# jiahuei/COMIC-Compact-Image-Captioning-with-Attention

Hardware: AMD Instinct MI355X
Metric: images/sec (decoder-mode XE training, COMIC-256, InceptionV3 frozen) (higher is better)
Workload: dtype bf16

## Files before the change

### comic-compact-image-captioning-with-attention_amd/csrc/gemm_group.hip

```cpp
#include <algorithm>

#include "gemm_group.h"
#include "gemm_x3_dev.h"

namespace {

constexpr int GB = 128;
constexpr int kGemmGroupSlots = 512;
constexpr int kItemOverhead = 6;
constexpr int kSc1 = 16;
typedef __attribute__((ext_vector_type(4))) unsigned gg_u32x4_t;

__device__ __forceinline__ __amdgpu_buffer_rsrc_t gg_rsrc(const void* p, long bytes) {
  return __builtin_amdgcn_make_buffer_rsrc((void*)p, 0, (int)bytes, 0x00020000);
}
__device__ __forceinline__ float4 gg_load16_sc1(__amdgpu_buffer_rsrc_t r, unsigned off) {
  const gg_u32x4_t v = __builtin_amdgcn_raw_buffer_load_b128(r, (int)off, 0, kSc1);
  return make_float4(__uint_as_float(v.x), __uint_as_float(v.y), __uint_as_float(v.z), __uint_as_float(v.w));
}
__device__ __forceinline__ void gg_store16_sc1(__amdgpu_buffer_rsrc_t r, unsigned off, float4 v) {
  const gg_u32x4_t u = {__float_as_uint(v.x), __float_as_uint(v.y), __float_as_uint(v.z), __float_as_uint(v.w)};
  __builtin_amdgcn_raw_buffer_store_b128(u, r, (int)off, 0, kSc1);
}

constexpr int kGroupLds = 4 * (X3Tile<GB, true>::BYTES + X3Tile<GB, true>::BYTES);
static_assert(X3Tile<GB, true>::BYTES >= X3Tile<GB, false>::BYTES, "LDS of the k-contiguous form bounds the others");
constexpr int kGroupLdsPc = 2 * 2 * (X3TilePc<GB, false>::BYTES + X3TilePc<GB, false>::BYTES);
static_assert(X3TilePc<GB, false>::BYTES >= X3TilePc<GB, true>::BYTES, "LDS of the row-contiguous form bounds the others");

__device__ __forceinline__ void gg_emit(const ComicGemmProb& p, int m, int n, float4 a) {
  if (m >= p.M || n >= p.N) return;
  const int nv = min(4, p.N - n);
  float v[4] = {a.x * p.alpha, a.y * p.alpha, a.z * p.alpha, a.w * p.alpha};
  float* cp = p.C + (size_t)m * p.ldc + n;
#pragma unroll
  for (int q = 0; q < 4; ++q) {
    if (q >= nv) break;
    if (p.bias) v[q] += p.bias[n + q];
    if (p.mask) v[q] = (v[q] / p.keep) * p.mask[(size_t)m * p.ld_mask + n + q];
    if (p.beta != 0.f) v[q] += p.beta * cp[q];
  }
  if (nv == 4 && (p.ldc % 4 == 0) && (((uintptr_t)p.C & 15) == 0)) {
    *(float4*)cp = make_float4(v[0], v[1], v[2], v[3]);
  } else {
#pragma unroll
    for (int q = 0; q < 4; ++q)
      if (q < nv) cp[q] = v[q];
  }
}

template <int FORM>
__global__ __launch_bounds__(FORM == 1 ? 256 : 512)
#if defined(__HIP_DEVICE_COMPILE__)
__attribute__((amdgpu_waves_per_eu(FORM == 3 ? 4 : 1, FORM == 3 ? 4 : 2)))
#endif
void gemm_group_x3_kernel(ComicGemmGroup g) {
  constexpr bool PC = FORM != 1;
  constexpr int NT = PC ? 512 : 256;
  constexpr int LDS = PC ? kGroupLdsPc : kGroupLds;
  extern __shared__ __attribute__((aligned(16))) unsigned char smem[];
  int bid = blockIdx.x;
  if (g.xcd_chunk > 0 && bid < g.xcd_chunk * 8) bid = (bid & 7) * g.xcd_chunk + (bid >> 3);
  volatile unsigned* s_last = (volatile unsigned*)(smem + LDS - 16);
  int pi = 0;
#pragma unroll 1
  for (int i = 1; i < g.n; ++i)
    if (bid >= g.p[i].wg_begin) pi = i;
  const ComicGemmProb& p = g.p[pi];
  const int local = bid - p.wg_begin;
  const int S = p.S, ntiles = p.tiles_m * p.tiles_n;
  const int slice = local / ntiles, tl = local - slice * ntiles;
  constexpr int PW = 8;
  const int panel = tl / (p.tiles_m * PW), rem = tl - panel * p.tiles_m * PW;
  const int pw = min(PW, p.tiles_n - panel * PW);
  const int mt = rem / pw, nt = panel * PW + rem % pw;
  const int tile = mt * p.tiles_n + nt;
  const int m0 = mt * GB, n0 = nt * GB;
  const int kbeg = S > 1 ? slice * p.k_per_slice : 0;
  const int kend = S > 1 ? min(p.K, kbeg + p.k_per_slice) : p.K;
  const int tid = threadIdx.x, lane = tid & 63, wave = tid >> 6;
  const int wm = wave >> 1, wn = wave & 1;

  const long tile_id = (long)p.ticket0 + tile;
  const __amdgpu_buffer_rsrc_t sr = gg_rsrc(g.slab + ((long)p.slab_tile0 + (long)tile * S) * (GB * GB), (long)S * GB * GB * 4);
  const unsigned sbase = (unsigned)slice * (GB * GB * 4);
  if (p.ones_a) {
    constexpr int KG = 8;
    float4* red = (float4*)smem;
    const int cg = tid & 31, kg = tid >> 5, n = n0 + 4 * cg;
    const bool vec = (p.ldb % 4 == 0) && (((uintptr_t)p.B & 15) == 0);
    float4 sm = make_float4(0.f, 0.f, 0.f, 0.f);
    if (n < p.N && kg < KG)
      for (int k = kbeg + kg; k < kend; k += KG) {
        const float4 v = load4(p.B + (size_t)k * p.ldb + n, p.N - n, vec);
        sm.x += v.x; sm.y += v.y; sm.z += v.z; sm.w += v.w;
      }
    if (kg < KG) red[kg * 32 + cg] = sm;
    __syncthreads();
    if (tid < 32) {
      float4 tot = red[cg];
#pragma unroll
      for (int k = 1; k < KG; ++k) {
        const float4 v = red[k * 32 + cg];
        tot.x += v.x; tot.y += v.y; tot.z += v.z; tot.w += v.w;
      }
      if (S == 1) gg_emit(p, 0, n, tot);
      else gg_store16_sc1(sr, sbase + (unsigned)cg * 16u, tot);
    }
    if (S == 1) return;
  } else {
    f32x4_t acc[4][4];
    if constexpr (PC) {
      constexpr int DEPTH = FORM == 3 ? 2 : 4;
      if (p.type == COMIC_GG_TN) x3_mainloop_pc<false, false, DEPTH>(p.A, p.B, p.M, p.N, p.lda, p.ldb, m0, n0, kbeg, kend, smem, acc);
      else if (p.type == COMIC_GG_NN) x3_mainloop_pc<true, false, DEPTH>(p.A, p.B, p.M, p.N, p.lda, p.ldb, m0, n0, kbeg, kend, smem, acc);
      else x3_mainloop_pc<true, true, DEPTH>(p.A, p.B, p.M, p.N, p.lda, p.ldb, m0, n0, kbeg, kend, smem, acc);
    } else {
      if (p.type == COMIC_GG_TN)
        x3_mainloop<GB, false, false, GB>(p.A, p.B, p.M, p.N, p.lda, p.ldb, m0, n0, kbeg, kend, smem, acc);
      else if (p.type == COMIC_GG_NN)
        x3_mainloop<GB, true, false, GB>(p.A, p.B, p.M, p.N, p.lda, p.ldb, m0, n0, kbeg, kend, smem, acc);
      else
        x3_mainloop<GB, true, true, GB>(p.A, p.B, p.M, p.N, p.lda, p.ldb, m0, n0, kbeg, kend, smem, acc);
    }
    const bool owner = wave < 4;
    if (S == 1) {
      if (owner)
#pragma unroll
      for (int i = 0; i < 4; ++i)
#pragma unroll
        for (int j = 0; j < 4; ++j)
          gg_emit(p, m0 + wm * 64 + j * 16 + (lane & 15), n0 + wn * 64 + i * 16 + (lane >> 4) * 4,
                  make_float4(acc[i][j][0], acc[i][j][1], acc[i][j][2], acc[i][j][3]));
      return;
    }
    if (owner)
#pragma unroll
    for (int i = 0; i < 4; ++i)
#pragma unroll
      for (int j = 0; j < 4; ++j) {
        const int ml = wm * 64 + j * 16 + (lane & 15), nl = wn * 64 + i * 16 + (lane >> 4) * 4;
        gg_store16_sc1(sr, sbase + (unsigned)(ml * GB + nl) * 4u, make_float4(acc[i][j][0], acc[i][j][1], acc[i][j][2], acc[i][j][3]));
      }
  }
  asm volatile("s_waitcnt vmcnt(0)" ::: "memory");
  __syncthreads();
  if (tid == 0) {
    const unsigned t = __hip_atomic_fetch_add(g.tickets + tile_id, 1u, __ATOMIC_RELAXED, __HIP_MEMORY_SCOPE_AGENT);
    *s_last = (t == (unsigned)(S - 1)) ? 1u : 0u;
    if (t == (unsigned)(S - 1)) __hip_atomic_store(g.tickets + tile_id, 0u, __ATOMIC_RELAXED, __HIP_MEMORY_SCOPE_AGENT);
  }
  __syncthreads();
  if (!*s_last) return;
  const int n_chunks = p.ones_a ? 1 : (GB * GB / 4) / NT;
#pragma unroll 1
  for (int c = 0; c < n_chunks; c += 4) {
    float4 sum[4];
#pragma unroll
    for (int u = 0; u < 4; ++u) sum[u] = make_float4(0.f, 0.f, 0.f, 0.f);
#pragma unroll 1
    for (int s = 0; s < S; ++s) {
      float4 v[4];
#pragma unroll
      for (int u = 0; u < 4; ++u) v[u] = gg_load16_sc1(sr, (unsigned)s * (GB * GB * 4) + (unsigned)(tid + NT * (c + u)) * 16u);
#pragma unroll
      for (int u = 0; u < 4; ++u) {
        sum[u].x += v[u].x; sum[u].y += v[u].y; sum[u].z += v[u].z; sum[u].w += v[u].w;
      }
    }
#pragma unroll
    for (int u = 0; u < 4; ++u) {
      const int idx4 = tid + NT * (c + u);
      if (!p.ones_a || idx4 < GB / 4) gg_emit(p, m0 + idx4 / (GB / 4), n0 + (idx4 % (GB / 4)) * 4, sum[u]);
    }
  }
}


}

int comic_gemm_group_plan(ComicGemmGroup& g, int target_items, int64_t* slab_bytes, int* n_tickets) {
  COMIC_REQUIRE(g.n > 0 && g.n <= kGemmGroupMax, "gemm_group: %d problems", g.n);
  long cost = 0;
  for (int i = 0; i < g.n; ++i) {
    ComicGemmProb& p = g.p[i];
    COMIC_REQUIRE(p.M > 0 && p.N > 0 && p.K > 0 && p.B && p.C && (p.A || p.ones_a), "gemm_group: bad problem %d", i);
    COMIC_REQUIRE(p.type >= COMIC_GG_TN && p.type <= COMIC_GG_NT, "gemm_group: bad type of problem %d", i);
    COMIC_REQUIRE(!p.ones_a || (p.type == COMIC_GG_TN && p.M == 1), "gemm_group: ones_a needs type TN and M = 1 (problem %d)", i);
    COMIC_REQUIRE(p.ldc >= p.N && (!p.mask || p.ld_mask >= p.N), "gemm_group: leading dimension of problem %d", i);
    if (!p.ones_a) COMIC_REQUIRE(p.lda >= (p.type == COMIC_GG_TN ? p.M : p.K), "gemm_group: lda of problem %d", i);
    COMIC_REQUIRE(p.ldb >= (p.type == COMIC_GG_NT ? p.K : p.N), "gemm_group: ldb of problem %d", i);
    p.tiles_m = cdiv(p.M, GB);
    p.tiles_n = cdiv(p.N, GB);
    cost += (long)cdiv(p.M, GB) * p.tiles_n * cdiv(p.K, 32);
  }
  auto split_of = [](int kt, long klen) { return (int)std::min<long>(16, std::max<long>(1, (kt + klen / 2) / klen)); };
  long klen = std::max<long>(8, cost / std::max(1, target_items));
  {
    long best = -1, best_klen = klen, kt_max = 8;
    for (int i = 0; i < g.n; ++i) kt_max = std::max<long>(kt_max, cdiv(g.p[i].K, 32));
    for (long kl = klen; kl <= kt_max; ++kl) {
      long items = 0, longest = 0;
      for (int i = 0; i < g.n; ++i) {
        const ComicGemmProb& p = g.p[i];
        const int kt = cdiv(p.K, 32), S = split_of(kt, kl);
        items += (long)p.tiles_m * p.tiles_n * S;
        if (!p.ones_a) longest = std::max<long>(longest, cdiv(kt, S));
      }
      const long est = cdiv64(items, kGemmGroupSlots) * (longest + kItemOverhead);
      if (best < 0 || est < best) {
        best = est;
        best_klen = kl;
      }
    }
    klen = best_klen;
  }
  int wg = 0, tickets = 0, slab_tiles = 0;
  for (int i = 0; i < g.n; ++i) {
    ComicGemmProb& p = g.p[i];
    const int nt = cdiv(p.M, GB) * p.tiles_n, kt = cdiv(p.K, 32);
    int S = split_of(kt, klen);
    p.k_per_slice = cdiv(kt, S) * 32;
    S = cdiv(p.K, p.k_per_slice);
    p.S = S;
    p.wg_begin = wg;
    p.slab_tile0 = slab_tiles;
    p.ticket0 = tickets;
    wg += nt * S;
    if (S > 1) {
      slab_tiles += nt * S;
      tickets += nt;
    }
  }
  if (slab_bytes) *slab_bytes = (int64_t)slab_tiles * GB * GB * 4;
  if (n_tickets) *n_tickets = tickets;
  return wg;
}

namespace {
bool gg_vec_ok(const ComicGemmGroup& g) {
  for (int i = 0; i < g.n; ++i) {
    const ComicGemmProb& p = g.p[i];
    if (p.ones_a) continue;
    const bool a_kc = p.type != COMIC_GG_TN, b_kc = p.type == COMIC_GG_NT;
    if (!(p.lda % 4 == 0 && p.ldb % 4 == 0 && ((uintptr_t)p.A & 15) == 0 && ((uintptr_t)p.B & 15) == 0 &&
          (!(a_kc || b_kc) || p.K % 4 == 0)))
      return false;
  }
  return true;
}
const void* gg_kernel(int form) {
  return form == 1 ? (const void*)gemm_group_x3_kernel<1> : form == 2 ? (const void*)gemm_group_x3_kernel<2> : (const void*)gemm_group_x3_kernel<3>;
}
int gg_lds(int form) { return form == 1 ? kGroupLds : kGroupLdsPc; }
int gg_reserve_lds(int form) {
  static PerDeviceOnce once[3];
  bool& done = once[form - 1].slot();
  if (!done) {
    COMIC_REQUIRE(hipFuncSetAttribute(gg_kernel(form), hipFuncAttributeMaxDynamicSharedMemorySize, gg_lds(form)) == hipSuccess,
                  "gemm_group: cannot reserve %d bytes of LDS", gg_lds(form));
    done = true;
  }
  return 0;
}
}

int comic_gemm_group_launch(const ComicGemmGroup& g_in, int n_wg, hipStream_t st, int form) {
  ComicGemmGroup g = g_in;
  g.xcd_chunk = n_wg / 8;
  COMIC_REQUIRE(n_wg > 0, "gemm_group: empty launch");
  COMIC_REQUIRE(form >= 0 && form <= 3, "gemm_group: form %d", form);
  const bool vec = gg_vec_ok(g);
  if (form == 0) form = vec ? 3 : 1;
  COMIC_REQUIRE(form == 1 || vec, "gemm_group: form %d needs 16-byte loadable operands", form);
  if (int rc = gg_reserve_lds(form)) return rc;
  if (form == 1) hipLaunchKernelGGL(gemm_group_x3_kernel<1>, dim3((unsigned)n_wg), dim3(256), kGroupLds, st, g);
  else if (form == 2) hipLaunchKernelGGL(gemm_group_x3_kernel<2>, dim3((unsigned)n_wg), dim3(512), kGroupLdsPc, st, g);
  else hipLaunchKernelGGL(gemm_group_x3_kernel<3>, dim3((unsigned)n_wg), dim3(512), kGroupLdsPc, st, g);
  COMIC_LAUNCH_CHECK("gemm_group");
  return 0;
}

namespace {
int gg_from_public(const comic_gemm_prob* probs, int n, ComicGemmGroup& g) {
  COMIC_REQUIRE(probs && n > 0 && n <= kGemmGroupMax, "gemm_group: 1..%d problems", kGemmGroupMax);
  g = ComicGemmGroup{};
  g.n = n;
  for (int i = 0; i < n; ++i) {
    const comic_gemm_prob& q = probs[i];
    ComicGemmProb& p = g.p[i];
    p.A = q.A; p.B = q.B; p.C = q.C; p.bias = q.bias; p.mask = q.mask;
    p.M = q.M; p.N = q.N; p.K = q.K; p.lda = q.lda; p.ldb = q.ldb; p.ldc = q.ldc; p.ld_mask = q.ld_mask;
    p.alpha = q.alpha; p.beta = q.beta; p.keep = q.keep; p.type = q.type; p.ones_a = q.ones_a;
  }
  return 0;
}
#define kPublicTarget kGemmGroupTargetItems
}

extern "C" int64_t comic_gemm_group_workspace(const comic_gemm_prob* probs, int n) {
  ComicGemmGroup g;
  if (gg_from_public(probs, n, g)) return -1;
  int64_t slab = 0;
  int nt = 0;
  if (comic_gemm_group_plan(g, kPublicTarget, &slab, &nt) < 0) return -1;
  return slab + 256 + (int64_t)nt * 4;
}

extern "C" int comic_gemm_group_form(const comic_gemm_prob* probs, int n, void* workspace, int64_t workspace_bytes, int form,
                                     void* stream) {
  COMIC_REQUIRE(form >= 0 && form <= 3, "gemm_group: form %d", form);
  ComicGemmGroup g;
  if (int rc = gg_from_public(probs, n, g)) return rc;
  int64_t slab = 0;
  int nt = 0;
  const int wg = comic_gemm_group_plan(g, kPublicTarget, &slab, &nt);
  if (wg < 0) return 2;
  COMIC_REQUIRE(form < 2 || gg_vec_ok(g), "gemm_group: form %d needs 16-byte loadable operands", form);
  const int64_t slab_al = (slab + 255) / 256 * 256;
  COMIC_REQUIRE(nt == 0 || (workspace && workspace_bytes >= slab_al + (int64_t)nt * 4), "gemm_group: workspace too small");
  g.slab = (float*)workspace;
  g.tickets = nt ? (unsigned*)((char*)workspace + slab_al) : nullptr;
  if (nt) COMIC_REQUIRE(hipMemsetAsync(g.tickets, 0, (size_t)nt * 4, (hipStream_t)stream) == hipSuccess, "gemm_group: memset");
  return comic_gemm_group_launch(g, wg, (hipStream_t)stream, form);
}

extern "C" int comic_gemm_group(const comic_gemm_prob* probs, int n, void* workspace, int64_t workspace_bytes, void* stream) {
  return comic_gemm_group_form(probs, n, workspace, workspace_bytes, 0, stream);
}

extern "C" int comic_gemm_group_resident(int form) {
  if (form < 1 || form > 3) {
    comic_set_error("gemm_group: form %d", form);
    return -1;
  }
  if (gg_reserve_lds(form)) return -1;
  int nb = 0;
  if (hipOccupancyMaxActiveBlocksPerMultiprocessor(&nb, gg_kernel(form), form == 1 ? 256 : 512, gg_lds(form)) != hipSuccess) {
    comic_set_error("gemm_group: occupancy query failed");
    return -1;
  }
  return nb;
}
```

### comic-compact-image-captioning-with-attention_amd/csrc/gemm_x3_dev.h

```cpp
#pragma once
#include <type_traits>

#include "common.h"

namespace {

__device__ __forceinline__ float4 load4(const float* __restrict__ p, int nvalid, bool vec_ok) {
  if (nvalid >= 4 && vec_ok) return *(const float4*)p;
  float4 r = make_float4(0.f, 0.f, 0.f, 0.f);
  if (nvalid > 0) r.x = p[0];
  if (nvalid > 1) r.y = p[1];
  if (nvalid > 2) r.z = p[2];
  if (nvalid > 3) r.w = p[3];
  return r;
}

__device__ __forceinline__ void split_bf16x2(float a, float b, uint32_t& hi, uint32_t& lo) {
  hi = pack_bf16x2(a, b);
  lo = pack_bf16x2(a - __uint_as_float(hi << 16), b - __uint_as_float(hi & 0xFFFF0000u));
}

template <int ROWS, bool KC>
struct X3Tile {
  static constexpr int ROWB = 80;
  static constexpr int KSTR = 2 * ROWS + 32;
  static constexpr int BYTES = KC ? ROWS * ROWB : 32 * KSTR;
};

template <int ROWS, bool KC>
__device__ __forceinline__ void x3_chunk(int q, int ld, int row0, int rows_total, int k0, int K, int& c, int& ext, int& nv,
                                         size_t& base) {
  int r, k;
  if (KC) {
    r = row0 + (q >> 3); k = k0 + (q & 7) * 4;
    c = k; ext = K; nv = r < rows_total ? K - k : 0;
    base = (size_t)min(r, rows_total - 1) * ld;
  } else {
    constexpr int CPR = ROWS / 4;
    k = k0 + q / CPR; r = row0 + (q % CPR) * 4;
    c = r; ext = rows_total; nv = k < K ? rows_total - r : 0;
    base = (size_t)min(k, K - 1) * ld;
  }
}
template <int ROWS, bool KC, int NCH, bool VEC>
__device__ __forceinline__ void x3_load_tile(const float* __restrict__ g, int ld, int row0, int rows_total, int k0, int K,
                                             int tid, float4 (&out)[NCH]) {
#pragma unroll
  for (int i = 0; i < NCH; ++i) {
    int c, ext, nv;
    size_t base;
    x3_chunk<ROWS, KC>(tid + 256 * i, ld, row0, rows_total, k0, K, c, ext, nv, base);
    const float* bp = g + base;
    if (VEC) {
      out[i] = *(const float4*)(bp + max(0, min(c, ext - 4)));
    } else {
      const int e = ext - 1;
      out[i] = make_float4(bp[min(c, e)], bp[min(c + 1, e)], bp[min(c + 2, e)], bp[min(c + 3, e)]);
    }
  }
}
template <int ROWS, bool KC, int NCH, bool VEC>
__device__ __forceinline__ void x3_mask_tile(int row0, int rows_total, int k0, int K, int tid, float4 (&v)[NCH]) {
#pragma unroll
  for (int i = 0; i < NCH; ++i) {
    int c, ext, nv;
    size_t base;
    x3_chunk<ROWS, KC>(tid + 256 * i, 0, row0, rows_total, k0, K, c, ext, nv, base);
    if (VEC) {
      const bool ok = nv >= 4;
      v[i].x = ok ? v[i].x : 0.f; v[i].y = ok ? v[i].y : 0.f; v[i].z = ok ? v[i].z : 0.f; v[i].w = ok ? v[i].w : 0.f;
    } else {
      v[i].x = nv > 0 ? v[i].x : 0.f; v[i].y = nv > 1 ? v[i].y : 0.f; v[i].z = nv > 2 ? v[i].z : 0.f; v[i].w = nv > 3 ? v[i].w : 0.f;
    }
  }
}
template <int ROWS, bool KC, int NCH>
__device__ __forceinline__ void x3_store_tile(unsigned char* hi_base, unsigned char* lo_base, int tid,
                                              const float4 (&in)[NCH]) {
  using T = X3Tile<ROWS, KC>;
#pragma unroll
  for (int i = 0; i < NCH; ++i) {
    const int q = tid + 256 * i;
    uint32_t h0, l0, h1, l1;
    split_bf16x2(in[i].x, in[i].y, h0, l0);
    split_bf16x2(in[i].z, in[i].w, h1, l1);
    int off;
    if (KC) {
      const int row = q >> 3, c = q & 7;
      off = row * T::ROWB + (2 * (c & 3) + (c >> 2)) * 8;
    } else {
      constexpr int CPR = ROWS / 4;
      const int kk = q / CPR, row = (q % CPR) * 4;
      off = kk * T::KSTR + row * 2;
    }
    *(uint2*)(hi_base + off) = make_uint2(h0, h1);
    *(uint2*)(lo_base + off) = make_uint2(l0, l1);
  }
}
typedef __attribute__((ext_vector_type(4))) short x3_s16x4_t;
typedef __attribute__((ext_vector_type(8))) short x3_s16x8_t;
template <int ROWS, bool KC>
__device__ __forceinline__ bf16x8_t x3_frag(const unsigned char* base, int row16, int lane) {
  using T = X3Tile<ROWS, KC>;
  if (KC) {
    const uint4 v = *(const uint4*)(base + (row16 + (lane & 15)) * T::ROWB + (lane >> 4) * 16);
    return __builtin_bit_cast(bf16x8_t, v);
  } else {
    const int g = lane >> 4, q = (lane >> 2) & 3, pp = lane & 3;
    const unsigned char* p = base + (4 * g + q) * T::KSTR + (row16 + 4 * pp) * 2;
    const uint32_t a0 = (uint32_t)(uintptr_t)((__attribute__((address_space(3))) const unsigned char*)p);
    const x3_s16x4_t lo = __builtin_amdgcn_ds_read_tr16_b64_v4i16((__attribute__((address_space(3))) x3_s16x4_t*)(uintptr_t)a0);
    const x3_s16x4_t hi =
        __builtin_amdgcn_ds_read_tr16_b64_v4i16((__attribute__((address_space(3))) x3_s16x4_t*)(uintptr_t)(a0 + 16 * T::KSTR));
    const x3_s16x8_t v = {lo[0], lo[1], lo[2], lo[3], hi[0], hi[1], hi[2], hi[3]};
    return __builtin_bit_cast(bf16x8_t, v);
  }
}


constexpr unsigned kOor = 0x80000000u;
template <int ROWS, bool KC, int NCH, bool VEC>
struct X3Src {
  const float* g;
  int ld, row0, rows_total, kend;
  __amdgpu_buffer_rsrc_t rs;
  unsigned base;
  unsigned rb[NCH];
  int kc;
  unsigned step8;
  __device__ __forceinline__ void init(const float* g_, int ld_, int row0_, int rows_total_, int kbeg, int kend_, int tid) {
    g = g_; ld = ld_; row0 = row0_; rows_total = rows_total_; kend = kend_;
    if (VEC) {
      rs = __builtin_amdgcn_make_buffer_rsrc((void*)g, 0, 0x7FFFFFF0, 0x00020000);
      if (KC) {
        kc = (tid & 7) * 4;
#pragma unroll
        for (int i = 0; i < NCH; ++i) {
          const int r = row0 + (tid >> 3) + 32 * i;
          rb[i] = r < rows_total ? (unsigned)(((long)r * ld + kc) * 4) : kOor;
        }
      } else {
        constexpr int CPR = ROWS / 4;
        const int r = row0 + (tid % CPR) * 4;
        const long rec = ((long)(kend - 1) * ld + min(ld, (rows_total + 3) & ~3)) * 4;
        rs = __builtin_amdgcn_make_buffer_rsrc((void*)g, 0, (int)rec, 0x00020000);
        base = r < rows_total ? (unsigned)(((long)(kbeg + tid / CPR) * ld + r) * 4) : kOor;
        step8 = (unsigned)((256 / CPR) * ld * 4);
      }
    }
  }
  __device__ __forceinline__ void load(int k0, int tid, float4 (&out)[NCH]) {
    if (VEC) {
      typedef __attribute__((ext_vector_type(4))) unsigned u4;
      if (KC) {
        const unsigned past = (unsigned)((kend - 1 - (k0 + kc)) >> 31) & kOor;
#pragma unroll
        for (int i = 0; i < NCH; ++i) {
          const unsigned o = (rb[i] + (unsigned)k0 * 4u) | past;
          const u4 v = __builtin_amdgcn_raw_buffer_load_b128(rs, (int)o, 0, 0);
          out[i] = make_float4(__uint_as_float(v.x), __uint_as_float(v.y), __uint_as_float(v.z), __uint_as_float(v.w));
        }
      } else if constexpr (256 % (ROWS / 4) == 0) {
#pragma unroll
        for (int i = 0; i < NCH; ++i) {
          const u4 v = __builtin_amdgcn_raw_buffer_load_b128(rs, (int)(base + (unsigned)i * step8), 0, 0);
          out[i] = make_float4(__uint_as_float(v.x), __uint_as_float(v.y), __uint_as_float(v.z), __uint_as_float(v.w));
        }
        base += (unsigned)(32 * ld * 4);
      } else {
        constexpr int CPR = ROWS / 4;
#pragma unroll
        for (int i = 0; i < NCH; ++i) {
          const int q = tid + 256 * i, r = row0 + (q % CPR) * 4;
          const unsigned o = r < rows_total ? (unsigned)(((long)(k0 + q / CPR) * ld + r) * 4) : kOor;
          const u4 v = __builtin_amdgcn_raw_buffer_load_b128(rs, (int)o, 0, 0);
          out[i] = make_float4(__uint_as_float(v.x), __uint_as_float(v.y), __uint_as_float(v.z), __uint_as_float(v.w));
        }
      }
    } else {
      x3_load_tile<ROWS, KC, NCH, false>(g, ld, row0, rows_total, k0, kend, tid, out);
    }
  }
  __device__ __forceinline__ void mask(int k0, int tid, float4 (&v)[NCH]) {
    if (!VEC) x3_mask_tile<ROWS, KC, NCH, false>(row0, rows_total, k0, kend, tid, v);
  }
};

template <int BM, bool A_KC, bool B_KC, int BN, bool VEC>
__device__ __forceinline__ void x3_mainloop_v(const float* __restrict__ A, const float* __restrict__ B, int M, int N, int lda,
                                            int ldb, int m0, int n0, int kbeg, int kend, unsigned char* smem,
                                            f32x4_t (&acc)[BN / 32][BM / 32]) {
  constexpr int BKx = 32;
  constexpr int TM = BM / 32, TN = BN / 32;
  constexpr int ACH = BM * BKx / 4 / 256, BCH = BN * BKx / 4 / 256;
  constexpr int ABYTES = X3Tile<BM, A_KC>::BYTES, BBYTES = X3Tile<BN, B_KC>::BYTES;
  unsigned char* Ah = smem;
  unsigned char* Al = Ah + 2 * ABYTES;
  unsigned char* Bh = Al + 2 * ABYTES;
  unsigned char* Bl = Bh + 2 * BBYTES;
  const int tid = threadIdx.x, lane = tid & 63, wave = tid >> 6;
  const int wm = wave >> 1, wn = wave & 1;
#pragma unroll
  for (int i = 0; i < TN; ++i)
#pragma unroll
    for (int j = 0; j < TM; ++j) acc[i][j] = (f32x4_t){0.f, 0.f, 0.f, 0.f};
  float4 ar[2][ACH], br[2][BCH];
  const int nk = ((kend - kbeg + BKx - 1) / BKx + 1) & ~1;
  X3Src<BM, A_KC, ACH, VEC> sa;
  X3Src<BN, B_KC, BCH, VEC> sb;
  sa.init(A, lda, m0, M, kbeg, kend, tid);
  sb.init(B, ldb, n0, N, kbeg, kend, tid);
  sa.load(kbeg, tid, ar[0]);
  sb.load(kbeg, tid, br[0]);
  sa.load(kbeg + BKx, tid, ar[1]);
  sb.load(kbeg + BKx, tid, br[1]);
  sa.mask(kbeg, tid, ar[0]);
  sb.mask(kbeg, tid, br[0]);
  x3_store_tile<BM, A_KC, ACH>(Ah, Al, tid, ar[0]);
  x3_store_tile<BN, B_KC, BCH>(Bh, Bl, tid, br[0]);
  __syncthreads();
  auto step = [&](const int kt, auto par) {
    constexpr int P = decltype(par)::value;
    sa.load(kbeg + (kt + 2) * BKx, tid, ar[P]);
    sb.load(kbeg + (kt + 2) * BKx, tid, br[P]);
    bf16x8_t bh[TN], bl[TN], ah[TM], al[TM];
#pragma unroll
    for (int i = 0; i < TN; ++i) {
      bh[i] = x3_frag<BN, B_KC>(Bh + P * BBYTES, wn * (BN / 2) + i * 16, lane);
      bl[i] = x3_frag<BN, B_KC>(Bl + P * BBYTES, wn * (BN / 2) + i * 16, lane);
    }
#pragma unroll
    for (int j = 0; j < TM; ++j) {
      ah[j] = x3_frag<BM, A_KC>(Ah + P * ABYTES, wm * (BM / 2) + j * 16, lane);
      al[j] = x3_frag<BM, A_KC>(Al + P * ABYTES, wm * (BM / 2) + j * 16, lane);
    }
#pragma unroll
    for (int i = 0; i < TN; ++i)
#pragma unroll
      for (int j = 0; j < TM; ++j) {
        acc[i][j] = __builtin_amdgcn_mfma_f32_16x16x32_bf16(bl[i], ah[j], acc[i][j], 0, 0, 0);
        acc[i][j] = __builtin_amdgcn_mfma_f32_16x16x32_bf16(bh[i], al[j], acc[i][j], 0, 0, 0);
        acc[i][j] = __builtin_amdgcn_mfma_f32_16x16x32_bf16(bh[i], ah[j], acc[i][j], 0, 0, 0);
      }
    sa.mask(kbeg + (kt + 1) * BKx, tid, ar[P ^ 1]);
    sb.mask(kbeg + (kt + 1) * BKx, tid, br[P ^ 1]);
    x3_store_tile<BM, A_KC, ACH>(Ah + (P ^ 1) * ABYTES, Al + (P ^ 1) * ABYTES, tid, ar[P ^ 1]);
    x3_store_tile<BN, B_KC, BCH>(Bh + (P ^ 1) * BBYTES, Bl + (P ^ 1) * BBYTES, tid, br[P ^ 1]);
#ifdef COMIC_X3_SCHED
    __builtin_amdgcn_sched_group_barrier(0x020, ACH + BCH, 0);
    __builtin_amdgcn_sched_group_barrier(0x100, 64, 0);
#pragma unroll
    for (int r = 0; r < TM * TN; ++r) {
      __builtin_amdgcn_sched_group_barrier(0x008, 3, 0);
      __builtin_amdgcn_sched_group_barrier(0x002, 9, 0);
      __builtin_amdgcn_sched_group_barrier(0x200, 1, 0);
    }
#endif
    __syncthreads();
  };
  for (int kt = 0; kt < nk; kt += 2) {
    step(kt, std::integral_constant<int, 0>());
    step(kt + 1, std::integral_constant<int, 1>());
  }
}

template <int BM, bool A_KC, bool B_KC, int BN>
__device__ __forceinline__ void x3_mainloop(const float* __restrict__ A, const float* __restrict__ B, int M, int N, int lda,
                                            int ldb, int m0, int n0, int kbeg, int kend, unsigned char* smem,
                                            f32x4_t (&acc)[BN / 32][BM / 32]) {
  const bool a_vec = (lda % 4 == 0) && (((uintptr_t)A & 15) == 0) && (!A_KC || kend % 4 == 0);
  const bool b_vec = (ldb % 4 == 0) && (((uintptr_t)B & 15) == 0) && (!B_KC || kend % 4 == 0);
  if (a_vec && b_vec) x3_mainloop_v<BM, A_KC, B_KC, BN, true>(A, B, M, N, lda, ldb, m0, n0, kbeg, kend, smem, acc);
  else x3_mainloop_v<BM, A_KC, B_KC, BN, false>(A, B, M, N, lda, ldb, m0, n0, kbeg, kend, smem, acc);
}

template <int ROWS, bool KC>
struct X3TilePc {
  static constexpr int KSTR = 2 * ROWS + 32;
  static constexpr int BYTES = KC ? ROWS * 64 : 32 * KSTR;
};
__device__ __forceinline__ int x3_swz(int row) { return (0x6C >> (((row >> 2) & 3) * 2)) & 3; }

template <int ROWS, bool KC, int NCH, bool TIGHT = false>
__device__ __forceinline__ void x3pc_store_tile(unsigned char* hi_base, unsigned char* lo_base, int tid,
                                                const float4 (&in)[NCH]) {
  using T = X3TilePc<ROWS, KC>;
#pragma unroll
  for (int i = 0; i < NCH; ++i) {
    if (TIGHT) __builtin_amdgcn_sched_barrier(0);
    const int q = tid + 256 * i;
    uint32_t h0, l0, h1, l1;
    split_bf16x2(in[i].x, in[i].y, h0, l0);
    split_bf16x2(in[i].z, in[i].w, h1, l1);
    int off;
    if (KC) {
      const int row = q >> 3, c = q & 7;
      off = row * 64 + (((c & 3) ^ x3_swz(row)) * 2 + (c >> 2)) * 8;
    } else {
      constexpr int CPR = ROWS / 4;
      const int kk = q / CPR, row = (q % CPR) * 4;
      off = kk * T::KSTR + row * 2;
    }
    *(uint2*)(hi_base + off) = make_uint2(h0, h1);
    *(uint2*)(lo_base + off) = make_uint2(l0, l1);
  }
}
template <int ROWS, bool KC>
__device__ __forceinline__ bf16x8_t x3pc_frag(const unsigned char* base, int row16, int lane) {
  using T = X3TilePc<ROWS, KC>;
  if (KC) {
    const int row = row16 + (lane & 15);
    const uint4 v = *(const uint4*)(base + row * 64 + (((lane >> 4) ^ x3_swz(row)) * 16));
    return __builtin_bit_cast(bf16x8_t, v);
  } else {
    const int g = lane >> 4, q = (lane >> 2) & 3, pp = lane & 3;
    const unsigned char* p = base + (4 * g + q) * T::KSTR + (row16 + 4 * pp) * 2;
    const uint32_t a0 = (uint32_t)(uintptr_t)((__attribute__((address_space(3))) const unsigned char*)p);
    const x3_s16x4_t lo = __builtin_amdgcn_ds_read_tr16_b64_v4i16((__attribute__((address_space(3))) x3_s16x4_t*)(uintptr_t)a0);
    const x3_s16x4_t hi =
        __builtin_amdgcn_ds_read_tr16_b64_v4i16((__attribute__((address_space(3))) x3_s16x4_t*)(uintptr_t)(a0 + 16 * T::KSTR));
    const x3_s16x8_t v = {lo[0], lo[1], lo[2], lo[3], hi[0], hi[1], hi[2], hi[3]};
    return __builtin_bit_cast(bf16x8_t, v);
  }
}

template <bool A_KC, bool B_KC, int DEPTH>
__device__ __forceinline__ void x3_mainloop_pc(const float* __restrict__ A, const float* __restrict__ B, int M, int N, int lda,
                                               int ldb, int m0, int n0, int kbeg, int kend, unsigned char* smem,
                                               f32x4_t (&acc)[4][4]) {
  static_assert(DEPTH == 2 || DEPTH == 4, "register sets of the producers");
  constexpr int BM = 128, BN = 128, BKx = 32, NCH = 4;
  constexpr int ABYTES = X3TilePc<BM, A_KC>::BYTES, BBYTES = X3TilePc<BN, B_KC>::BYTES;
  constexpr int STAGE = 2 * (ABYTES + BBYTES);
  const int tid = threadIdx.x, lane = tid & 63;
  const int wave = __builtin_amdgcn_readfirstlane(tid >> 6);
  const int nk = ((kend - kbeg + BKx - 1) / BKx + DEPTH - 1) & ~(DEPTH - 1);
  if (wave >= 4) {
    const int pt = tid - 256;
    X3Src<BM, A_KC, NCH, true> sa;
    X3Src<BN, B_KC, NCH, true> sb;
    sa.init(A, lda, m0, M, kbeg, kend, pt);
    sb.init(B, ldb, n0, N, kbeg, kend, pt);
    float4 ar[DEPTH][NCH], br[DEPTH][NCH];
#pragma unroll
    for (int s = 0; s < DEPTH; ++s) {
      sa.load(kbeg + s * BKx, pt, ar[s]);
      sb.load(kbeg + s * BKx, pt, br[s]);
    }
    auto put = [&](int stage, const float4 (&a)[NCH], const float4 (&b)[NCH]) {
      unsigned char* st = smem + stage * STAGE;
      x3pc_store_tile<BM, A_KC, NCH, DEPTH == 2>(st, st + ABYTES, pt, a);
      x3pc_store_tile<BN, B_KC, NCH, DEPTH == 2>(st + 2 * ABYTES, st + 2 * ABYTES + BBYTES, pt, b);
      if (DEPTH == 2) __builtin_amdgcn_sched_barrier(0);
    };
    put(0, ar[0], br[0]);
    sa.load(kbeg + DEPTH * BKx, pt, ar[0]);
    sb.load(kbeg + DEPTH * BKx, pt, br[0]);
    __syncthreads();
    auto step = [&](int kt, auto s_) {
      constexpr int S = decltype(s_)::value;
      put(S & 1, ar[S], br[S]);
      sa.load(kbeg + (kt + 1 + DEPTH) * BKx, pt, ar[S]);
      sb.load(kbeg + (kt + 1 + DEPTH) * BKx, pt, br[S]);
      __syncthreads();
    };
    for (int kt = 0; kt < nk; kt += DEPTH) {
      if constexpr (DEPTH == 4) {
        step(kt, std::integral_constant<int, 1>());
        step(kt + 1, std::integral_constant<int, 2>());
        step(kt + 2, std::integral_constant<int, 3>());
        step(kt + 3, std::integral_constant<int, 0>());
      } else {
        step(kt, std::integral_constant<int, 1>());
        step(kt + 1, std::integral_constant<int, 0>());
      }
    }
  } else {
    const int wm = wave >> 1, wn = wave & 1;
#pragma unroll
    for (int i = 0; i < 4; ++i)
#pragma unroll
      for (int j = 0; j < 4; ++j) acc[i][j] = (f32x4_t){0.f, 0.f, 0.f, 0.f};
    __syncthreads();
    auto step = [&](auto p_) {
      constexpr int P = decltype(p_)::value;
      const unsigned char* st = smem + P * STAGE;
      bf16x8_t ah[4], al[4];
#pragma unroll
      for (int j = 0; j < 4; ++j) {
        ah[j] = x3pc_frag<BM, A_KC>(st, wm * 64 + j * 16, lane);
        al[j] = x3pc_frag<BM, A_KC>(st + ABYTES, wm * 64 + j * 16, lane);
      }
      if constexpr (DEPTH == 4) {
        bf16x8_t bh[4], bl[4];
#pragma unroll
        for (int i = 0; i < 4; ++i) {
          bh[i] = x3pc_frag<BN, B_KC>(st + 2 * ABYTES, wn * 64 + i * 16, lane);
          bl[i] = x3pc_frag<BN, B_KC>(st + 2 * ABYTES + BBYTES, wn * 64 + i * 16, lane);
        }
#pragma unroll
        for (int i = 0; i < 4; ++i)
#pragma unroll
          for (int j = 0; j < 4; ++j) {
            acc[i][j] = __builtin_amdgcn_mfma_f32_16x16x32_bf16(bl[i], ah[j], acc[i][j], 0, 0, 0);
            acc[i][j] = __builtin_amdgcn_mfma_f32_16x16x32_bf16(bh[i], al[j], acc[i][j], 0, 0, 0);
            acc[i][j] = __builtin_amdgcn_mfma_f32_16x16x32_bf16(bh[i], ah[j], acc[i][j], 0, 0, 0);
          }
      } else {
        bf16x8_t bh[2], bl[2];
        bh[0] = x3pc_frag<BN, B_KC>(st + 2 * ABYTES, wn * 64, lane);
        bl[0] = x3pc_frag<BN, B_KC>(st + 2 * ABYTES + BBYTES, wn * 64, lane);
#pragma unroll
        for (int i = 0; i < 4; ++i) {
          if (i < 3) {
            bh[(i + 1) & 1] = x3pc_frag<BN, B_KC>(st + 2 * ABYTES, wn * 64 + (i + 1) * 16, lane);
            bl[(i + 1) & 1] = x3pc_frag<BN, B_KC>(st + 2 * ABYTES + BBYTES, wn * 64 + (i + 1) * 16, lane);
          }
#pragma unroll
          for (int j = 0; j < 4; ++j) {
            acc[i][j] = __builtin_amdgcn_mfma_f32_16x16x32_bf16(bl[i & 1], ah[j], acc[i][j], 0, 0, 0);
            acc[i][j] = __builtin_amdgcn_mfma_f32_16x16x32_bf16(bh[i & 1], al[j], acc[i][j], 0, 0, 0);
            acc[i][j] = __builtin_amdgcn_mfma_f32_16x16x32_bf16(bh[i & 1], ah[j], acc[i][j], 0, 0, 0);
          }
          __builtin_amdgcn_sched_barrier(0);
        }
      }
      __syncthreads();
    };
    for (int kt = 0; kt < nk; kt += 2) {
      step(std::integral_constant<int, 0>());
      step(std::integral_constant<int, 1>());
    }
  }
}

}
```

Measured before the change: 40210.

## Add DMA-to-LDS grouped GEMM form with five-slot ring pipeline for small launches

Adds a fourth grouped-GEMM kernel form that streams raw fp32 operand tiles straight into LDS with buffer_load_lds into a five-slot ring, then splits them to bf16 hi/lo fragments at read time for the 3-MFMA emulated fp32 product. All 8 waves compute a 2x4 layout of 64x32 subtiles, so no waves sit idle. The default dispatch picks this form when the launch has at most 256 workgroups. The aim is to cut register-staged global loads and overlap memory with MFMA on small grouped GEMMs, at the cost of a smaller k-tile and per-iteration barriers.

```diff
diff --git a/comic-compact-image-captioning-with-attention_amd/csrc/gemm_group.hip b/comic-compact-image-captioning-with-attention_amd/csrc/gemm_group.hip
--- a/comic-compact-image-captioning-with-attention_amd/csrc/gemm_group.hip
+++ b/comic-compact-image-captioning-with-attention_amd/csrc/gemm_group.hip
@@ -9,6 +9,7 @@
 constexpr int kGemmGroupSlots = 512;
 constexpr int kItemOverhead = 6;
 constexpr int kSc1 = 16;
+constexpr int kDmaMaxItems = kGemmGroupSlots / 2;
 typedef __attribute__((ext_vector_type(4))) unsigned gg_u32x4_t;
 
 __device__ __forceinline__ __amdgpu_buffer_rsrc_t gg_rsrc(const void* p, long bytes) {
@@ -27,6 +28,8 @@
 static_assert(X3Tile<GB, true>::BYTES >= X3Tile<GB, false>::BYTES, "LDS of the k-contiguous form bounds the others");
 constexpr int kGroupLdsPc = 2 * 2 * (X3TilePc<GB, false>::BYTES + X3TilePc<GB, false>::BYTES);
 static_assert(X3TilePc<GB, false>::BYTES >= X3TilePc<GB, true>::BYTES, "LDS of the row-contiguous form bounds the others");
+constexpr int kDmaSlots = 5;
+constexpr int kGroupLdsDma = kDmaSlots * kX3RawTile;
 
 __device__ __forceinline__ void gg_emit(const ComicGemmProb& p, int m, int n, float4 a) {
   if (m >= p.M || n >= p.N) return;
@@ -52,12 +55,14 @@
 template <int FORM>
 __global__ __launch_bounds__(FORM == 1 ? 256 : 512)
 #if defined(__HIP_DEVICE_COMPILE__)
-__attribute__((amdgpu_waves_per_eu(FORM == 3 ? 4 : 1, FORM == 3 ? 4 : 2)))
+__attribute__((amdgpu_waves_per_eu(FORM >= 3 ? 4 : 1, FORM >= 3 ? 4 : 2)))
 #endif
 void gemm_group_x3_kernel(ComicGemmGroup g) {
-  constexpr bool PC = FORM != 1;
-  constexpr int NT = PC ? 512 : 256;
-  constexpr int LDS = PC ? kGroupLdsPc : kGroupLds;
+  constexpr bool DMA = FORM == 4;
+  constexpr bool PC = FORM == 2 || FORM == 3;
+  constexpr int NT = FORM == 1 ? 256 : 512;
+  constexpr int LDS = DMA ? kGroupLdsDma : PC ? kGroupLdsPc : kGroupLds;
+  constexpr int TNW = DMA ? 2 : 4;
   extern __shared__ __attribute__((aligned(16))) unsigned char smem[];
   int bid = blockIdx.x;
   if (g.xcd_chunk > 0 && bid < g.xcd_chunk * 8) bid = (bid & 7) * g.xcd_chunk + (bid >> 3);
@@ -79,7 +84,7 @@
   const int kbeg = S > 1 ? slice * p.k_per_slice : 0;
   const int kend = S > 1 ? min(p.K, kbeg + p.k_per_slice) : p.K;
   const int tid = threadIdx.x, lane = tid & 63, wave = tid >> 6;
-  const int wm = wave >> 1, wn = wave & 1;
+  const int wm = DMA ? wave >> 2 : wave >> 1, wn = DMA ? wave & 3 : wave & 1;
 
   const long tile_id = (long)p.ticket0 + tile;
   const __amdgpu_buffer_rsrc_t sr = gg_rsrc(g.slab + ((long)p.slab_tile0 + (long)tile * S) * (GB * GB), (long)S * GB * GB * 4);
@@ -109,8 +114,12 @@
     }
     if (S == 1) return;
   } else {
-    f32x4_t acc[4][4];
-    if constexpr (PC) {
+    f32x4_t acc[TNW][4];
+    if constexpr (DMA) {
+      if (p.type == COMIC_GG_TN) x3_mainloop_dma<false, false, kDmaSlots>(p.A, p.B, p.M, p.N, p.lda, p.ldb, m0, n0, kbeg, kend, smem, acc);
+      else if (p.type == COMIC_GG_NN) x3_mainloop_dma<true, false, kDmaSlots>(p.A, p.B, p.M, p.N, p.lda, p.ldb, m0, n0, kbeg, kend, smem, acc);
+      else x3_mainloop_dma<true, true, kDmaSlots>(p.A, p.B, p.M, p.N, p.lda, p.ldb, m0, n0, kbeg, kend, smem, acc);
+    } else if constexpr (PC) {
       constexpr int DEPTH = FORM == 3 ? 2 : 4;
       if (p.type == COMIC_GG_TN) x3_mainloop_pc<false, false, DEPTH>(p.A, p.B, p.M, p.N, p.lda, p.ldb, m0, n0, kbeg, kend, smem, acc);
       else if (p.type == COMIC_GG_NN) x3_mainloop_pc<true, false, DEPTH>(p.A, p.B, p.M, p.N, p.lda, p.ldb, m0, n0, kbeg, kend, smem, acc);
@@ -123,23 +132,23 @@
       else
         x3_mainloop<GB, true, true, GB>(p.A, p.B, p.M, p.N, p.lda, p.ldb, m0, n0, kbeg, kend, smem, acc);
     }
-    const bool owner = wave < 4;
+    const bool owner = DMA || wave < 4;
     if (S == 1) {
       if (owner)
 #pragma unroll
-      for (int i = 0; i < 4; ++i)
+      for (int i = 0; i < TNW; ++i)
 #pragma unroll
         for (int j = 0; j < 4; ++j)
-          gg_emit(p, m0 + wm * 64 + j * 16 + (lane & 15), n0 + wn * 64 + i * 16 + (lane >> 4) * 4,
+          gg_emit(p, m0 + wm * 64 + j * 16 + (lane & 15), n0 + wn * (16 * TNW) + i * 16 + (lane >> 4) * 4,
                   make_float4(acc[i][j][0], acc[i][j][1], acc[i][j][2], acc[i][j][3]));
       return;
     }
     if (owner)
 #pragma unroll
-    for (int i = 0; i < 4; ++i)
+    for (int i = 0; i < TNW; ++i)
 #pragma unroll
       for (int j = 0; j < 4; ++j) {
-        const int ml = wm * 64 + j * 16 + (lane & 15), nl = wn * 64 + i * 16 + (lane >> 4) * 4;
+        const int ml = wm * 64 + j * 16 + (lane & 15), nl = wn * (16 * TNW) + i * 16 + (lane >> 4) * 4;
         gg_store16_sc1(sr, sbase + (unsigned)(ml * GB + nl) * 4u, make_float4(acc[i][j][0], acc[i][j][1], acc[i][j][2], acc[i][j][3]));
       }
   }
@@ -250,11 +259,14 @@
   return true;
 }
 const void* gg_kernel(int form) {
-  return form == 1 ? (const void*)gemm_group_x3_kernel<1> : form == 2 ? (const void*)gemm_group_x3_kernel<2> : (const void*)gemm_group_x3_kernel<3>;
-}
-int gg_lds(int form) { return form == 1 ? kGroupLds : kGroupLdsPc; }
+  return form == 1   ? (const void*)gemm_group_x3_kernel<1>
+         : form == 2 ? (const void*)gemm_group_x3_kernel<2>
+         : form == 3 ? (const void*)gemm_group_x3_kernel<3>
+                     : (const void*)gemm_group_x3_kernel<4>;
+}
+int gg_lds(int form) { return form == 1 ? kGroupLds : form == 4 ? kGroupLdsDma : kGroupLdsPc; }
 int gg_reserve_lds(int form) {
-  static PerDeviceOnce once[3];
+  static PerDeviceOnce once[4];
   bool& done = once[form - 1].slot();
   if (!done) {
     COMIC_REQUIRE(hipFuncSetAttribute(gg_kernel(form), hipFuncAttributeMaxDynamicSharedMemorySize, gg_lds(form)) == hipSuccess,
@@ -269,14 +281,15 @@
   ComicGemmGroup g = g_in;
   g.xcd_chunk = n_wg / 8;
   COMIC_REQUIRE(n_wg > 0, "gemm_group: empty launch");
-  COMIC_REQUIRE(form >= 0 && form <= 3, "gemm_group: form %d", form);
+  COMIC_REQUIRE(form >= 0 && form <= 4, "gemm_group: form %d", form);
   const bool vec = gg_vec_ok(g);
-  if (form == 0) form = vec ? 3 : 1;
+  if (form == 0) form = !vec ? 1 : n_wg <= kDmaMaxItems ? 4 : 3;
   COMIC_REQUIRE(form == 1 || vec, "gemm_group: form %d needs 16-byte loadable operands", form);
   if (int rc = gg_reserve_lds(form)) return rc;
   if (form == 1) hipLaunchKernelGGL(gemm_group_x3_kernel<1>, dim3((unsigned)n_wg), dim3(256), kGroupLds, st, g);
   else if (form == 2) hipLaunchKernelGGL(gemm_group_x3_kernel<2>, dim3((unsigned)n_wg), dim3(512), kGroupLdsPc, st, g);
-  else hipLaunchKernelGGL(gemm_group_x3_kernel<3>, dim3((unsigned)n_wg), dim3(512), kGroupLdsPc, st, g);
+  else if (form == 3) hipLaunchKernelGGL(gemm_group_x3_kernel<3>, dim3((unsigned)n_wg), dim3(512), kGroupLdsPc, st, g);
+  else hipLaunchKernelGGL(gemm_group_x3_kernel<4>, dim3((unsigned)n_wg), dim3(512), kGroupLdsDma, st, g);
   COMIC_LAUNCH_CHECK("gemm_group");
   return 0;
 }
@@ -309,7 +322,7 @@
 
 extern "C" int comic_gemm_group_form(const comic_gemm_prob* probs, int n, void* workspace, int64_t workspace_bytes, int form,
                                      void* stream) {
-  COMIC_REQUIRE(form >= 0 && form <= 3, "gemm_group: form %d", form);
+  COMIC_REQUIRE(form >= 0 && form <= 4, "gemm_group: form %d", form);
   ComicGemmGroup g;
   if (int rc = gg_from_public(probs, n, g)) return rc;
   int64_t slab = 0;
@@ -330,7 +343,7 @@
 }
 
 extern "C" int comic_gemm_group_resident(int form) {
-  if (form < 1 || form > 3) {
+  if (form < 1 || form > 4) {
     comic_set_error("gemm_group: form %d", form);
     return -1;
   }
diff --git a/comic-compact-image-captioning-with-attention_amd/csrc/gemm_x3_dev.h b/comic-compact-image-captioning-with-attention_amd/csrc/gemm_x3_dev.h
--- a/comic-compact-image-captioning-with-attention_amd/csrc/gemm_x3_dev.h
+++ b/comic-compact-image-captioning-with-attention_amd/csrc/gemm_x3_dev.h
@@ -434,4 +434,186 @@
   }
 }
 
-}
+constexpr int kX3RawTile = 128 * 32 * 4;
+
+template <int OFF>
+__device__ __forceinline__ float x3_lds_read32(uint32_t addr) {
+  float v;
+  asm volatile("ds_read_b32 %0, %1 offset:%2" : "=v"(v) : "v"(addr), "i"(OFF));
+  return v;
+}
+template <int OFF>
+__device__ __forceinline__ void x3_lds_read128(uint32_t addr, float (&v)[4]) {
+  typedef __attribute__((ext_vector_type(4))) float f4;
+  f4 t;
+  asm volatile("ds_read_b128 %0, %1 offset:%2" : "=v"(t) : "v"(addr), "i"(OFF));
+  v[0] = t[0]; v[1] = t[1]; v[2] = t[2]; v[3] = t[3];
+}
+template <int N>
+__device__ __forceinline__ void x3_wait_vmcnt() {
+  asm volatile("s_waitcnt vmcnt(%0)" ::"i"(N) : "memory");
+}
+
+template <bool KC>
+struct X3DmaSrc {
+  __amdgpu_buffer_rsrc_t rs;
+  unsigned off[2];
+  unsigned step;
+  int kc, kend;
+  __device__ __forceinline__ void init(const float* g, int ld, int row0, int rows_total, int kbeg, int kend_, int wave, int lane) {
+    kend = kend_;
+    if (KC) {
+      rs = __builtin_amdgcn_make_buffer_rsrc((void*)g, 0, 0x7FFFFFF0, 0x00020000);
+      kc = ((lane & 7) ^ ((4 * (wave & 1) + (lane >> 4)) & 7)) * 4;
+#pragma unroll
+      for (int i = 0; i < 2; ++i) {
+        const int r = row0 + 8 * wave + 64 * i + (lane >> 3);
+        off[i] = r < rows_total ? (unsigned)(((long)r * ld + kc) * 4) : kOor;
+      }
+    } else {
+      const long rec = ((long)(kend - 1) * ld + min(ld, (rows_total + 3) & ~3)) * 4;
+      rs = __builtin_amdgcn_make_buffer_rsrc((void*)g, 0, (int)rec, 0x00020000);
+      const int r = row0 + 4 * ((lane & 31) ^ (4 * ((wave >> 1) & 1)));
+#pragma unroll
+      for (int i = 0; i < 2; ++i)
+        off[i] = r < rows_total ? (unsigned)(((long)(kbeg + 2 * wave + 16 * i + (lane >> 5)) * ld + r) * 4) : kOor;
+      step = (unsigned)(32 * ld * 4);
+    }
+  }
+  __device__ __forceinline__ void issue(int k0, unsigned char* tile, int wave) {
+    const unsigned past = KC ? (unsigned)((kend - 1 - (k0 + kc)) >> 31) & kOor : 0u;
+#pragma unroll
+    for (int i = 0; i < 2; ++i) {
+      const unsigned o = KC ? ((off[i] + (unsigned)k0 * 4u) | past) : off[i];
+      __builtin_amdgcn_raw_ptr_buffer_load_lds(rs, (__attribute__((address_space(3))) void*)(tile + (wave + 8 * i) * 1024), 16, (int)o, 0, 0, 0);
+      if (!KC) off[i] += step;
+    }
+  }
+};
+
+template <bool KC>
+struct X3DmaFrag {
+  uint32_t a0, a1;
+  __device__ __forceinline__ void init(int wb, int lane) {
+    const int r = lane & 15, g = lane >> 4;
+    if (KC) {
+      a0 = (uint32_t)((wb + r) * 128 + ((g ^ (r >> 1)) & 7) * 16);
+      a1 = a0 ^ 64u;
+    } else {
+      const uint32_t b = (uint32_t)(4 * g * 512 + (wb + r) * 4);
+      a0 = b + 64u * (g & 1);
+      a1 = b + 64u * ((g & 1) ^ 1);
+    }
+  }
+  template <int JJ>
+  __device__ __forceinline__ void read(uint32_t img, float (&v)[8]) const {
+    if (KC) {
+      float lo4[4], hi4[4];
+      x3_lds_read128<JJ * 2048>(img + a0, lo4);
+      x3_lds_read128<JJ * 2048>(img + a1, hi4);
+#pragma unroll
+      for (int q = 0; q < 4; ++q) { v[q] = lo4[q]; v[4 + q] = hi4[q]; }
+    } else {
+      const uint32_t a = img + ((JJ & 1) ? a1 : a0);
+      constexpr int O = 128 * (JJ >> 1);
+      v[0] = x3_lds_read32<O>(a);
+      v[1] = x3_lds_read32<O + 512>(a);
+      v[2] = x3_lds_read32<O + 1024>(a);
+      v[3] = x3_lds_read32<O + 1536>(a);
+      v[4] = x3_lds_read32<O + 8192>(a);
+      v[5] = x3_lds_read32<O + 8192 + 512>(a);
+      v[6] = x3_lds_read32<O + 8192 + 1024>(a);
+      v[7] = x3_lds_read32<O + 8192 + 1536>(a);
+    }
+  }
+};
+__device__ __forceinline__ void x3_split_frag(const float (&v)[8], bf16x8_t& hi, bf16x8_t& lo) {
+  typedef __attribute__((ext_vector_type(4))) unsigned u4;
+  uint32_t h[4], l[4];
+#pragma unroll
+  for (int q = 0; q < 4; ++q) split_bf16x2(v[2 * q], v[2 * q + 1], h[q], l[q]);
+  hi = __builtin_bit_cast(bf16x8_t, (u4){h[0], h[1], h[2], h[3]});
+  lo = __builtin_bit_cast(bf16x8_t, (u4){l[0], l[1], l[2], l[3]});
+}
+
+template <bool A_KC, bool B_KC, int SLOTS>
+__device__ __forceinline__ void x3_mainloop_dma(const float* __restrict__ A, const float* __restrict__ B, int M, int N, int lda,
+                                                int ldb, int m0, int n0, int kbeg, int kend, unsigned char* smem,
+                                                f32x4_t (&acc)[2][4]) {
+  static_assert(SLOTS >= 4, "the two operand tiles being multiplied and the two being replaced");
+  constexpr int BKx = 32, LPO = 2;
+  const int lane = threadIdx.x & 63;
+  const int wave = __builtin_amdgcn_readfirstlane(threadIdx.x >> 6);
+  const int wm = wave >> 2, wn = wave & 3;
+  const int nkt = (kend - kbeg + BKx - 1) / BKx;
+#pragma unroll
+  for (int i = 0; i < 2; ++i)
+#pragma unroll
+    for (int j = 0; j < 4; ++j) acc[i][j] = (f32x4_t){0.f, 0.f, 0.f, 0.f};
+  X3DmaSrc<A_KC> sa;
+  X3DmaSrc<B_KC> sb;
+  sa.init(A, lda, m0, M, kbeg, kend, wave, lane);
+  sb.init(B, ldb, n0, N, kbeg, kend, wave, lane);
+  X3DmaFrag<A_KC> fa;
+  X3DmaFrag<B_KC> fb;
+  fa.init(wm * 64, lane);
+  fb.init(wn * 32, lane);
+  const uint32_t lds0 = (uint32_t)(uintptr_t)((__attribute__((address_space(3))) unsigned char*)smem);
+  int ws = 0, ka = kbeg, kb = kbeg;
+  auto issue_a = [&]() {
+    sa.issue(ka, smem + ws * kX3RawTile, wave);
+    ka += BKx;
+    ws = ws + 1 == SLOTS ? 0 : ws + 1;
+  };
+  auto issue_b = [&]() {
+    sb.issue(kb, smem + ws * kX3RawTile, wave);
+    kb += BKx;
+    ws = ws + 1 == SLOTS ? 0 : ws + 1;
+  };
+#pragma unroll
+  for (int u = 0; u < SLOTS - 2; ++u) {
+    if (u & 1) issue_b();
+    else issue_a();
+  }
+  int ra = 0, rb = 1;
+#pragma unroll 1
+  for (int kt = 0; kt < nkt; ++kt) {
+    x3_wait_vmcnt<(SLOTS - 4) * LPO>();
+    __builtin_amdgcn_s_barrier();
+    if constexpr (SLOTS & 1) {
+      issue_b();
+      issue_a();
+    } else {
+      issue_a();
+      issue_b();
+    }
+    const uint32_t ia = lds0 + ra * kX3RawTile, ib = lds0 + rb * kX3RawTile;
+    float vb[2][8], va[4][8];
+    fb.template read<0>(ib, vb[0]);
+    fb.template read<1>(ib, vb[1]);
+    fa.template read<0>(ia, va[0]);
+    fa.template read<1>(ia, va[1]);
+    fa.template read<2>(ia, va[2]);
+    fa.template read<3>(ia, va[3]);
+    asm volatile("s_waitcnt lgkmcnt(0)" ::: "memory");
+    __builtin_amdgcn_sched_barrier(0);
+    bf16x8_t bh[2], bl[2], ah[4], al[4];
+#pragma unroll
+    for (int i = 0; i < 2; ++i) x3_split_frag(vb[i], bh[i], bl[i]);
+#pragma unroll
+    for (int j = 0; j < 4; ++j) x3_split_frag(va[j], ah[j], al[j]);
+#pragma unroll
+    for (int i = 0; i < 2; ++i)
+#pragma unroll
+      for (int j = 0; j < 4; ++j) {
+        acc[i][j] = __builtin_amdgcn_mfma_f32_16x16x32_bf16(bl[i], ah[j], acc[i][j], 0, 0, 0);
+        acc[i][j] = __builtin_amdgcn_mfma_f32_16x16x32_bf16(bh[i], al[j], acc[i][j], 0, 0, 0);
+        acc[i][j] = __builtin_amdgcn_mfma_f32_16x16x32_bf16(bh[i], ah[j], acc[i][j], 0, 0, 0);
+      }
+    ra = ra + 2 >= SLOTS ? ra + 2 - SLOTS : ra + 2;
+    rb = rb + 2 >= SLOTS ? rb + 2 - SLOTS : rb + 2;
+  }
+  x3_wait_vmcnt<0>();
+}
+
+}
```

Result: no change. 40120 (-0.2%).
